# zhaotudou/HeteroFusionRCNN

Measured on AMD Instinct MI355X. Metric: KITTI frames/sec RPN train step, higher is better.
Workload: dtype f32; 1 GPU; RPN train step, hf/configs/rpn_multiclass.config: PointCNN 5 xconv (K=8; 16384/4096/1024/256/64 points; C 256..1024, X-transformation, global branch) + 6 xdconv layers + fc 256/256, 3 classes, seg head, projection of the points into the image + gather of the image feature map (B,360,1200,32) + path drop 0.9/0.9 + 'concat' fusion, bin-based box head (fc 512/512, 3x76 outputs), targets + focal/softm; frames_per_gpu=8, global_batch=8, parallelism=dp1, hip_graph=True, optimizer=hf, x_branch_on_side_stream=True, scaling=strong, library_gemm_selection=library default heuristic, gradient_exchange=none (1 rank), geometry_prefetch_depth=2, geometry_prefetch_group=12

## Files before the change

heterofusionrcnn_amd/csrc/xconv.hip:

```cpp
#include "hf_common.h"

#include <initializer_list>

namespace hf {

template <int M>
__device__ __forceinline__ void store_m(float *base, size_t elem, const float (&v)[M])
{
    float *p = base + elem;
    if constexpr (M == 4 || M == 8) {
        if ((reinterpret_cast<uintptr_t>(base) & 15) == 0) {
#pragma unroll
            for (int q = 0; q < M / 4; ++q) reinterpret_cast<float4 *>(p)[q] = make_float4(v[4 * q], v[4 * q + 1], v[4 * q + 2], v[4 * q + 3]);
            return;
        }
    } else if constexpr (M == 2) {
        if ((reinterpret_cast<uintptr_t>(base) & 7) == 0) { *reinterpret_cast<float2 *>(p) = make_float2(v[0], v[1]); return; }
    }
#pragma unroll
    for (int m = 0; m < M; ++m) p[m] = v[m];
}
template <int M>
__device__ __forceinline__ void load_m(const float *base, size_t elem, float (&v)[M])
{
    const float *p = base + elem;
    if constexpr (M == 4 || M == 8) {
        if ((reinterpret_cast<uintptr_t>(base) & 15) == 0) {
#pragma unroll
            for (int q = 0; q < M / 4; ++q) {
                const float4 t = reinterpret_cast<const float4 *>(p)[q];
                v[4 * q] = t.x; v[4 * q + 1] = t.y; v[4 * q + 2] = t.z; v[4 * q + 3] = t.w;
            }
            return;
        }
    } else if constexpr (M == 2) {
        if ((reinterpret_cast<uintptr_t>(base) & 7) == 0) { const float2 t = *reinterpret_cast<const float2 *>(p); v[0] = t.x; v[1] = t.y; return; }
    }
#pragma unroll
    for (int m = 0; m < M; ++m) v[m] = p[m];
}


constexpr int kXcThreads = 256;

template <int K, bool TRANSPOSED>
__global__ __launch_bounds__(kXcThreads) void xconv_apply_kernel(long long rows, int c, const float *__restrict__ x,
                                                                const float *__restrict__ f, float *__restrict__ out)
{
    const int lane = threadIdx.x & 63;
    const long long wave = __builtin_amdgcn_readfirstlane(static_cast<int>(threadIdx.x >> 6)) +
                           static_cast<long long>(blockIdx.x) * (kXcThreads / 64);
    const long long nwaves = static_cast<long long>(gridDim.x) * (kXcThreads / 64);
    for (long long r = wave; r < rows; r += nwaves) {
        const float *xr = x + r * (K * K);
        float coef[K][K];
#pragma unroll
        for (int i = 0; i < K; ++i)
#pragma unroll
            for (int j = 0; j < K; ++j) coef[i][j] = TRANSPOSED ? xr[j * K + i] : xr[i * K + j];
        const float *fr = f + r * K * c;
        float *orow = out + r * K * c;
        for (int ch = lane; ch < c; ch += 64) {
            float v[K];
#pragma unroll
            for (int j = 0; j < K; ++j) v[j] = fr[static_cast<size_t>(j) * c + ch];
#pragma unroll
            for (int i = 0; i < K; ++i) {
                float acc = coef[i][0] * v[0];
#pragma unroll
                for (int j = 1; j < K; ++j) acc = acc + coef[i][j] * v[j];
                orow[static_cast<size_t>(i) * c + ch] = acc;
            }
        }
    }
}

template <int K>
__global__ __launch_bounds__(kXcThreads) void xconv_dx_kernel(long long rows, int c, const float *__restrict__ grad_out,
                                                             const float *__restrict__ f, float *__restrict__ grad_x)
{
    extern __shared__ float lds[];
    constexpr int KK = K * K, STRIDE = KK + 1;
    const int lane = threadIdx.x & 63, w = threadIdx.x >> 6;
    float *mine = lds + static_cast<size_t>(w) * 64 * STRIDE;
    const long long wave = w + static_cast<long long>(blockIdx.x) * (kXcThreads / 64);
    const long long nwaves = static_cast<long long>(gridDim.x) * (kXcThreads / 64);
    for (long long r = wave; r < rows; r += nwaves) {
        const float *gr = grad_out + r * K * c;
        const float *fr = f + r * K * c;
        float acc[K][K];
#pragma unroll
        for (int i = 0; i < K; ++i)
#pragma unroll
            for (int j = 0; j < K; ++j) acc[i][j] = 0.f;
        for (int ch = lane; ch < c; ch += 64) {
            float g[K], v[K];
#pragma unroll
            for (int j = 0; j < K; ++j) { g[j] = gr[static_cast<size_t>(j) * c + ch]; v[j] = fr[static_cast<size_t>(j) * c + ch]; }
#pragma unroll
            for (int i = 0; i < K; ++i)
#pragma unroll
                for (int j = 0; j < K; ++j) acc[i][j] = acc[i][j] + g[i] * v[j];
        }
#pragma unroll
        for (int i = 0; i < K; ++i)
#pragma unroll
            for (int j = 0; j < K; ++j) mine[lane * STRIDE + i * K + j] = acc[i][j];
        __builtin_amdgcn_fence(__ATOMIC_SEQ_CST, "wavefront");
        __builtin_amdgcn_wave_barrier();
        for (int p = lane; p < KK; p += 64) {
            float s = 0.f;
            for (int l = 0; l < 64; ++l) s = s + mine[l * STRIDE + p];
            grad_x[r * KK + p] = s;
        }
        __builtin_amdgcn_fence(__ATOMIC_SEQ_CST, "wavefront");
        __builtin_amdgcn_wave_barrier();
    }
}

template <int K, int M>
__global__ __launch_bounds__(kXcThreads) void depthwise_fwd_kernel(long long rows, int c, const float *__restrict__ x,
                                                                  const float *__restrict__ wgt, float *__restrict__ y)
{
    const long long total = rows * c;
    for (long long g = static_cast<long long>(blockIdx.x) * kXcThreads + threadIdx.x; g < total;
         g += static_cast<long long>(gridDim.x) * kXcThreads) {
        const long long r = g / c;
        const int ch = static_cast<int>(g - r * c);
        float acc[M];
#pragma unroll
        for (int m = 0; m < M; ++m) acc[m] = 0.f;
#pragma unroll
        for (int w = 0; w < K; ++w) {
            const float xv = x[(r * K + w) * c + ch];
#pragma unroll
            for (int m = 0; m < M; ++m) acc[m] = acc[m] + xv * wgt[(static_cast<size_t>(w) * c + ch) * M + m];
        }
        store_m<M>(y, static_cast<size_t>(g) * M, acc);
    }
}

template <int K, int M>
__global__ __launch_bounds__(kXcThreads) void depthwise_dx_kernel(long long rows, int c, const float *__restrict__ grad_y,
                                                                 const float *__restrict__ wgt, float *__restrict__ grad_x)
{
    const long long total = rows * c;
    for (long long g = static_cast<long long>(blockIdx.x) * kXcThreads + threadIdx.x; g < total;
         g += static_cast<long long>(gridDim.x) * kXcThreads) {
        const long long r = g / c;
        const int ch = static_cast<int>(g - r * c);
        float gy[M];
        load_m<M>(grad_y, static_cast<size_t>(g) * M, gy);
#pragma unroll
        for (int w = 0; w < K; ++w) {
            float acc = 0.f;
#pragma unroll
            for (int m = 0; m < M; ++m) acc = acc + gy[m] * wgt[(static_cast<size_t>(w) * c + ch) * M + m];
            grad_x[(r * K + w) * c + ch] = acc;
        }
    }
}

template <int K, int M, bool DX>
__global__ __launch_bounds__(kXcThreads) void depthwise_narrow_kernel(long long rows, int c, const float *__restrict__ in,
                                                                     const float *__restrict__ wgt, float *__restrict__ out)
{
    const long long tid = static_cast<long long>(blockIdx.x) * kXcThreads + threadIdx.x;
    const long long nthreads = static_cast<long long>(gridDim.x) * kXcThreads;
    const int ch = static_cast<int>(tid % c);
    float wr[K][M];
#pragma unroll
    for (int w = 0; w < K; ++w)
#pragma unroll
        for (int m = 0; m < M; ++m) wr[w][m] = wgt[(static_cast<size_t>(w) * c + ch) * M + m];
    for (long long r = tid / c; r < rows; r += nthreads / c) {
        if (!DX) {
            float acc[M];
#pragma unroll
            for (int m = 0; m < M; ++m) acc[m] = 0.f;
#pragma unroll
            for (int w = 0; w < K; ++w) {
                const float xv = in[(r * K + w) * c + ch];
#pragma unroll
                for (int m = 0; m < M; ++m) acc[m] = acc[m] + xv * wr[w][m];
            }
            store_m<M>(out, static_cast<size_t>(r * c + ch) * M, acc);
        } else {
            float gy[M];
            load_m<M>(in, static_cast<size_t>(r * c + ch) * M, gy);
#pragma unroll
            for (int w = 0; w < K; ++w) {
                float acc = 0.f;
#pragma unroll
                for (int m = 0; m < M; ++m) acc = acc + gy[m] * wr[w][m];
                out[(r * K + w) * c + ch] = acc;
            }
        }
    }
}

static int narrow_grid(long long rows, int c)
{
    int a = c, b = kXcThreads;
    while (b) { const int tmp = a % b; a = b; b = tmp; }
    const int unit = c / a;
    long long g = (rows * c + kXcThreads - 1) / kXcThreads;
    const long long cap = static_cast<long long>(kNumCU) * 8;
    if (g > cap) g = cap;
    g = (g + unit - 1) / unit * unit;
    return static_cast<int>(g);
}
constexpr int kNarrowMaxC = 64;

template <int K, int M>
__global__ __launch_bounds__(kXcThreads) void depthwise_dw_kernel(long long rows, int c, int rows_per_chunk,
                                                                 const float *__restrict__ x, const float *__restrict__ grad_y,
                                                                 float *__restrict__ grad_w, float *__restrict__ partial)
{
    extern __shared__ float red[];
    const int cw = c < kXcThreads ? c : kXcThreads, nrs = kXcThreads / cw;
    const int t = static_cast<int>(threadIdx.x);
    const int cl = t % cw, ch = blockIdx.x * cw + cl, rs = t / cw;
    const bool live = ch < c && rs < nrs;
    if (nrs > 1) {
        for (int i = t; i < K * M * cw; i += kXcThreads) red[i] = 0.f;
        __syncthreads();
    }
    const long long r0 = static_cast<long long>(blockIdx.y) * rows_per_chunk + rs;
    const long long r1 = static_cast<long long>(blockIdx.y + 1) * rows_per_chunk < rows ? static_cast<long long>(blockIdx.y + 1) * rows_per_chunk : rows;
    float acc[K][M];
#pragma unroll
    for (int w = 0; w < K; ++w)
#pragma unroll
        for (int m = 0; m < M; ++m) acc[w][m] = 0.f;
    if (live) {
        for (long long r = r0; r < r1; r += nrs) {
            float gy[M];
            load_m<M>(grad_y, static_cast<size_t>(r * c + ch) * M, gy);
#pragma unroll
            for (int w = 0; w < K; ++w) {
                const float xv = x[(r * K + w) * c + ch];
#pragma unroll
                for (int m = 0; m < M; ++m) acc[w][m] = acc[w][m] + xv * gy[m];
            }
        }
    }
    float *mine = partial ? partial + static_cast<size_t>(blockIdx.y) * K * c * M : nullptr;
    if (nrs == 1) {
        if (live) {
#pragma unroll
            for (int w = 0; w < K; ++w)
#pragma unroll
                for (int m = 0; m < M; ++m) {
                    const size_t e = (static_cast<size_t>(w) * c + ch) * M + m;
                    if (mine) mine[e] = acc[w][m];
                    else atomicAdd(&grad_w[e], acc[w][m]);
                }
        }
        return;
    }
    const bool shuffle = (cw & (cw - 1)) == 0 && cw <= 32;
    if (shuffle) {
        const int lane = t & 63, wave = t >> 6;
        __syncthreads();
#pragma unroll
        for (int w = 0; w < K; ++w)
#pragma unroll
            for (int m = 0; m < M; ++m) {
                float v = live ? acc[w][m] : 0.f;
                for (int off = cw; off < 64; off <<= 1) v += __shfl_xor(v, off);
                if (lane < cw) red[(wave * K * M + w * M + m) * cw + lane] = v;
            }
        __syncthreads();
        for (int i = t; i < K * M * cw; i += kXcThreads) {
            float v = red[i];
#pragma unroll
            for (int wv = 1; wv < kXcThreads / 64; ++wv) v += red[wv * K * M * cw + i];
            const int wm = i / cw, c2 = blockIdx.x * cw + i % cw;
            if (c2 < c) {
                const size_t e = (static_cast<size_t>(wm / M) * c + c2) * M + wm % M;
                if (mine) mine[e] = v;
                else atomicAdd(&grad_w[e], v);
            }
        }
        return;
    }
    if (live) {
#pragma unroll
        for (int w = 0; w < K; ++w)
#pragma unroll
            for (int m = 0; m < M; ++m) atomicAdd(&red[(w * M + m) * cw + cl], acc[w][m]);
    }
    __syncthreads();
    for (int i = t; i < K * M * cw; i += kXcThreads) {
        const int wm = i / cw, c2 = blockIdx.x * cw + i % cw;
        if (c2 < c) {
            const size_t e = (static_cast<size_t>(wm / M) * c + c2) * M + wm % M;
            if (mine) mine[e] = red[i];
            else atomicAdd(&grad_w[e], red[i]);
        }
    }
}

typedef float f2 __attribute__((ext_vector_type(2)));

struct XcPair {
    const float *base;
    unsigned hi;
    bool gathered, live, hi_live;
};

__device__ __forceinline__ XcPair xc_pair(int ch, int c, int c0, const float *f, const float *fts, bool gather)
{
    XcPair s;
    s.live = ch < c;
    s.hi_live = ch + 1 < c;
    const int cc = s.live ? ch : (c - 1) & ~1;
    s.hi = s.hi_live ? 1u : 0u;
    s.gathered = gather && cc >= c0;
    s.base = s.gathered ? fts + (cc - c0) : f + cc;
    return s;
}

template <bool V2>
__device__ __forceinline__ f2 ld_pair(const float *p, unsigned hi)
{
    if constexpr (V2) return *reinterpret_cast<const f2 *>(p);
    else return f2{p[0], p[hi]};
}

template <int M, bool V2>
__device__ __forceinline__ void st_pair_m(float *p, bool hi_live, const f2 (&v)[M])
{
    if constexpr (V2) {
#pragma unroll
        for (int q = 0; q < M; ++q) {
            const int e0 = 2 * q, e1 = 2 * q + 1;
            reinterpret_cast<f2 *>(p)[q] = f2{e0 < M ? v[e0].x : v[e0 - M].y, e1 < M ? v[e1].x : v[e1 - M].y};
        }
    } else {
#pragma unroll
        for (int m = 0; m < M; ++m) p[m] = v[m].x;
        if (hi_live) {
#pragma unroll
            for (int m = 0; m < M; ++m) p[M + m] = v[m].y;
        }
    }
}

constexpr int kXcRows = 2;

struct XcCloud {
    long long next;
    unsigned tbase;
};

__device__ __forceinline__ unsigned xc_tbase(XcCloud &cl, long long r, int rows_per_cloud, int n_src)
{
    while (r >= cl.next) { cl.next += rows_per_cloud; cl.tbase += static_cast<unsigned>(n_src); }
    return cl.tbase;
}

__device__ __forceinline__ XcCloud xc_cloud(long long r, int rows_per_cloud, int n_src)
{
    const long long b = r / rows_per_cloud;
    return XcCloud{(b + 1) * rows_per_cloud, static_cast<unsigned>(b * n_src)};
}

template <int K, bool GATHER, bool V2>
__device__ __forceinline__ void xc_gather_row(const XcPair &s, long long r, unsigned tbase, const int *__restrict__ idx,
                                              unsigned lstride, unsigned c1, f2 (&fv)[K])
{
    const unsigned rk = static_cast<unsigned>(r) * K;
#pragma unroll
    for (int j = 0; j < K; ++j) {
        const unsigned lo = (rk + j) * lstride;
        unsigned off = lo;
        if constexpr (GATHER) {
            const unsigned go = (tbase + static_cast<unsigned>(idx[rk + j])) * c1;
            off = s.gathered ? go : lo;
        }
        fv[j] = ld_pair<V2>(s.base + off, s.hi);
    }
}

template <int K>
struct XcXRows {
    static constexpr int KK = K * K, Q = (KK + 63) / 64;
    float v[kXcRows][Q];
    __device__ __forceinline__ void load(const float *__restrict__ x, const long long (&rr)[kXcRows], int lane)
    {
#pragma unroll
        for (int i = 0; i < kXcRows; ++i)
#pragma unroll
            for (int q = 0; q < Q; ++q) {
                const int p = lane + 64 * q;
                v[i][q] = x[rr[i] * KK + (p < KK ? p : KK - 1)];
            }
    }
    __device__ __forceinline__ void stage(float (*xs)[KK], int lane) const
    {
        __builtin_amdgcn_fence(__ATOMIC_SEQ_CST, "wavefront");
        __builtin_amdgcn_wave_barrier();
#pragma unroll
        for (int i = 0; i < kXcRows; ++i)
#pragma unroll
            for (int q = 0; q < Q; ++q)
                if (lane + 64 * q < KK) xs[i][lane + 64 * q] = v[i][q];
        __builtin_amdgcn_fence(__ATOMIC_SEQ_CST, "wavefront");
        __builtin_amdgcn_wave_barrier();
    }
};

template <int K, int M, bool GATHER, bool V2>
__global__ __launch_bounds__(kXcThreads) void xconv_dw_fwd_kernel(long long rows, int c, int c0, int rows_per_block,
                                                                 const float *__restrict__ x, const float *__restrict__ f,
                                                                 const float *__restrict__ fts, const int *__restrict__ idx, int n_src,
                                                                 int rows_per_cloud, const float *__restrict__ wd, float *__restrict__ out)
{
    const int lane = threadIdx.x & 63, wave = __builtin_amdgcn_readfirstlane(static_cast<int>(threadIdx.x >> 6));
    const int ch = blockIdx.y * 128 + 2 * lane;
    const XcPair src = xc_pair(ch, c, c0, f, fts, GATHER);
    const int cw = src.live ? ch : (c - 1) & ~1;
    f2 w[K][M];
#pragma unroll
    for (int k = 0; k < K; ++k)
#pragma unroll
        for (int m = 0; m < M; ++m) w[k][m] = f2{wd[(static_cast<size_t>(k) * c + cw) * M + m], wd[(static_cast<size_t>(k) * c + cw + src.hi) * M + m]};
    const unsigned lstride = GATHER ? c0 : c, c1 = c - c0;
    const long long r0 = static_cast<long long>(blockIdx.x) * rows_per_block;
    const long long r1 = r0 + rows_per_block < rows ? r0 + rows_per_block : rows;
    __shared__ float xs[kXcThreads / 64][kXcRows][K * K];
    XcCloud cl = xc_cloud(r0, rows_per_cloud, n_src);
    for (long long rb = r0 + wave; rb < r1; rb += 4 * kXcRows) {
        f2 fv[kXcRows][K];
        long long rr[kXcRows];
#pragma unroll
        for (int i = 0; i < kXcRows; ++i) rr[i] = rb + 4 * i < r1 ? rb + 4 * i : r1 - 1;
        XcXRows<K> xrow;
        xrow.load(x, rr, lane);
#pragma unroll
        for (int i = 0; i < kXcRows; ++i) {
            const unsigned tb = GATHER ? xc_tbase(cl, rr[i], rows_per_cloud, n_src) : 0u;
            xc_gather_row<K, GATHER, V2>(src, rr[i], tb, idx, lstride, c1, fv[i]);
        }
        xrow.stage(xs[wave], lane);
#pragma unroll
        for (int i = 0; i < kXcRows; ++i) {
            if (rb + 4 * i >= r1) break;
            const float *xr = xs[wave][i];
            f2 o[M];
#pragma unroll
            for (int m = 0; m < M; ++m) o[m] = f2{0.f, 0.f};
#pragma unroll
            for (int k = 0; k < K; ++k) {
                f2 t = xr[k * K] * fv[i][0];
#pragma unroll
                for (int j = 1; j < K; ++j) t = t + xr[k * K + j] * fv[i][j];
#pragma unroll
                for (int m = 0; m < M; ++m) o[m] = o[m] + t * w[k][m];
            }
            if (src.live) st_pair_m<M, V2>(out + static_cast<size_t>(rr[i] * c + ch) * M, src.hi_live, o);
        }
    }
}

struct XcSource {
    const float *base;
    long long stride;
    bool gathered;
};

__device__ __forceinline__ XcSource xc_source(int ch, int c, int c0, const float *f, const float *fts, const int *idx)
{
    XcSource s;
    if (idx == nullptr) { s.base = f + ch; s.stride = c; s.gathered = false; }
    else if (ch - (ch & 63) < c0) { s.base = f + ch; s.stride = c0; s.gathered = false; }
    else { s.base = fts + (ch - c0); s.stride = c - c0; s.gathered = true; }
    return s;
}

template <int K, int M, bool GATHER>
__global__ __launch_bounds__(kXcThreads) void xconv_dw_bwd_fw_kernel(long long rows, int c, int c0, int rows_per_block,
                                                                    const float *__restrict__ x, const float *__restrict__ f,
                                                                    const float *__restrict__ fts, const int *__restrict__ idx, int n_src,
                                                                    int rows_per_cloud, const float *__restrict__ wd,
                                                                    const float *__restrict__ grad_out, float *__restrict__ grad_f,
                                                                    float *__restrict__ grad_gathered, float *__restrict__ grad_wd,
                                                                    float *__restrict__ wd_partial)
{
    const int lane = threadIdx.x & 63, wave = __builtin_amdgcn_readfirstlane(static_cast<int>(threadIdx.x >> 6));
    const int ch = blockIdx.y * 64 + lane;
    const bool live = ch < c;
    const XcSource src = xc_source(live ? ch : blockIdx.y * 64, c, c0, f, fts, GATHER ? idx : nullptr);
    if (GATHER && src.gathered && !grad_wd && !grad_gathered) return;
    float w[K][M], gw[K][M];
#pragma unroll
    for (int k = 0; k < K; ++k)
#pragma unroll
        for (int m = 0; m < M; ++m) { w[k][m] = live ? wd[(static_cast<size_t>(k) * c + ch) * M + m] : 0.f; gw[k][m] = 0.f; }
    const long long r0 = static_cast<long long>(blockIdx.x) * rows_per_block;
    const long long r1 = r0 + rows_per_block < rows ? r0 + rows_per_block : rows;
    for (long long r = r0 + wave; r < r1; r += kXcThreads / 64) {
        const float *xr = x + r * (K * K);
        float fv[K], g[M], gfx[K];
        const long long tbase = (GATHER && src.gathered) ? static_cast<long long>(static_cast<unsigned>(r) / static_cast<unsigned>(rows_per_cloud)) * n_src : 0;
#pragma unroll
        for (int j = 0; j < K; ++j) {
            const long long srow = (GATHER && src.gathered) ? tbase + idx[r * K + j] : r * K + j;
            fv[j] = live ? src.base[srow * src.stride] : 0.f;
        }
        load_m<M>(grad_out, static_cast<size_t>(r * c + (live ? ch : 0)) * M, g);
        if (!live) {
#pragma unroll
            for (int m = 0; m < M; ++m) g[m] = 0.f;
        }
#pragma unroll
        for (int k = 0; k < K; ++k) {
            float a = 0.f;
#pragma unroll
            for (int m = 0; m < M; ++m) a = a + g[m] * w[k][m];
            gfx[k] = a;
            float t = xr[k * K] * fv[0];
#pragma unroll
            for (int j = 1; j < K; ++j) t = t + xr[k * K + j] * fv[j];
#pragma unroll
            for (int m = 0; m < M; ++m) gw[k][m] = gw[k][m] + t * g[m];
        }
        float *gdst = (GATHER && src.gathered) ? (grad_gathered ? grad_gathered + (ch - c0) : nullptr) : (grad_f ? grad_f + ch : nullptr);
        if (live && gdst) {
#pragma unroll
            for (int j = 0; j < K; ++j) {
                float a = xr[j] * gfx[0];
#pragma unroll
                for (int k = 1; k < K; ++k) a = a + xr[k * K + j] * gfx[k];
                gdst[(r * K + j) * src.stride] = a;
            }
        }
    }
    if (grad_wd) {
        __shared__ float red[K * M][64];
        for (int i = threadIdx.x; i < K * M * 64; i += kXcThreads) (&red[0][0])[i] = 0.f;
        __syncthreads();
        if (live) {
#pragma unroll
            for (int k = 0; k < K; ++k)
#pragma unroll
                for (int m = 0; m < M; ++m) atomicAdd(&red[k * M + m][lane], gw[k][m]);
        }
        __syncthreads();
        float *mine = wd_partial ? wd_partial + static_cast<size_t>(blockIdx.x) * K * c * M : nullptr;
        for (int i = threadIdx.x; i < K * M * 64; i += kXcThreads) {
            const int km = i >> 6, c2 = blockIdx.y * 64 + (i & 63);
            if (c2 < c) {
                const size_t e = (static_cast<size_t>(km / M) * c + c2) * M + km % M;
                if (mine) mine[e] = red[km][i & 63];
                else atomicAdd(&grad_wd[e], red[km][i & 63]);
            }
        }
    }
}

template <int K, int M, bool GATHER>
__global__ __launch_bounds__(kXcThreads) void xconv_dw_bwd_x_kernel(long long rows, int c, int c0, const float *__restrict__ f,
                                                                   const float *__restrict__ fts, const int *__restrict__ idx, int n_src,
                                                                   int rows_per_cloud, const float *__restrict__ wd,
                                                                   const float *__restrict__ grad_out, float *__restrict__ grad_x)
{
    extern __shared__ float lds[];
    constexpr int KK = K * K, STRIDE = KK + 1, QUADS = 16;
    const int lane = threadIdx.x & 63, w = threadIdx.x >> 6;
    float *mine = lds + static_cast<size_t>(w) * QUADS * STRIDE;
    const long long wave = w + static_cast<long long>(blockIdx.x) * (kXcThreads / 64);
    const long long nwaves = static_cast<long long>(gridDim.x) * (kXcThreads / 64);
    const int c1 = c - c0;
    for (long long r = wave; r < rows; r += nwaves) {
        float acc[K][K];
#pragma unroll
        for (int i = 0; i < K; ++i)
#pragma unroll
            for (int j = 0; j < K; ++j) acc[i][j] = 0.f;
        long long trow[K];
        if constexpr (GATHER) {
            const long long tbase = static_cast<long long>(static_cast<unsigned>(r) / static_cast<unsigned>(rows_per_cloud)) * n_src;
#pragma unroll
            for (int j = 0; j < K; ++j) trow[j] = tbase + idx[r * K + j];
        }
        for (int ch = lane; ch < c; ch += 64) {
            float fv[K], g[M];
            if constexpr (GATHER) {
                const bool gathered = ch >= c0;
                const float *base = gathered ? fts + (ch - c0) : f + ch;
                const long long stride = gathered ? c1 : c0;
#pragma unroll
                for (int j = 0; j < K; ++j) fv[j] = base[(gathered ? trow[j] : r * K + j) * stride];
            } else {
#pragma unroll
                for (int j = 0; j < K; ++j) fv[j] = f[(r * K + j) * c + ch];
            }
            load_m<M>(grad_out, static_cast<size_t>(r * c + ch) * M, g);
#pragma unroll
            for (int k = 0; k < K; ++k) {
                float a = 0.f;
#pragma unroll
                for (int m = 0; m < M; ++m) a = a + g[m] * wd[(static_cast<size_t>(k) * c + ch) * M + m];
#pragma unroll
                for (int j = 0; j < K; ++j) acc[k][j] = acc[k][j] + a * fv[j];
            }
        }
#pragma unroll
        for (int i = 0; i < K; ++i)
#pragma unroll
            for (int j = 0; j < K; ++j) {
                float v = acc[i][j];
                v = v + __int_as_float(__builtin_amdgcn_mov_dpp(__float_as_int(v), 0xb1, 0xf, 0xf, true));
                v = v + __int_as_float(__builtin_amdgcn_mov_dpp(__float_as_int(v), 0x4e, 0xf, 0xf, true));
                if ((lane & 3) == 0) mine[(lane >> 2) * STRIDE + i * K + j] = v;
            }
        __builtin_amdgcn_fence(__ATOMIC_SEQ_CST, "wavefront");
        __builtin_amdgcn_wave_barrier();
        for (int p = lane; p < KK; p += 64) {
            float s = 0.f;
#pragma unroll
            for (int l = 0; l < QUADS; ++l) s = s + mine[l * STRIDE + p];
            grad_x[r * KK + p] = s;
        }
        __builtin_amdgcn_fence(__ATOMIC_SEQ_CST, "wavefront");
        __builtin_amdgcn_wave_barrier();
    }
}

template <int K, int M>
__global__ __launch_bounds__(kXcThreads) void xconv_dw_bwd_fts_kernel(long long src_rows, int n_src, long long rows_per_cloud,
                                                                     int c, int c0, int rows_per_block,
                                                                     const float *__restrict__ x, const float *__restrict__ wd,
                                                                     const float *__restrict__ grad_out,
                                                                     const int *__restrict__ offsets, const int *__restrict__ entries,
                                                                     float *__restrict__ grad_fts)
{
    const int lane = threadIdx.x & 63, wave = __builtin_amdgcn_readfirstlane(static_cast<int>(threadIdx.x >> 6));
    const int c1 = c - c0, cf = blockIdx.y * 64 + lane, ch = c0 + cf;
    const bool live = cf < c1;
    float w[K][M];
#pragma unroll
    for (int k = 0; k < K; ++k)
#pragma unroll
        for (int m = 0; m < M; ++m) w[k][m] = live ? wd[(static_cast<size_t>(k) * c + ch) * M + m] : 0.f;
    const long long s0 = static_cast<long long>(blockIdx.x) * rows_per_block;
    const long long s1 = s0 + rows_per_block < src_rows ? s0 + rows_per_block : src_rows;
    long long bb = s0 / n_src;
    for (long long s = s0 + wave; s < s1; s += kXcThreads / 64) {
        while (s >= (bb + 1) * n_src) ++bb;
        const int pt = static_cast<int>(s - bb * n_src);
        const int *off = offsets + bb * (n_src + 1);
        const int *ent = entries + bb * rows_per_cloud * K;
        const int lo = off[pt], hi = off[pt + 1];
        float acc = 0.f;
        for (int e = lo; e < hi; e += 4) {
            float a4[4];
#pragma unroll
            for (int u = 0; u < 4; ++u) {
                const bool valid = e + u < hi;
                const int slot = ent[valid ? e + u : lo];
                const long long r = bb * rows_per_cloud + slot / K;
                const int j = slot % K;
                const float *xr = x + r * (K * K);
                float g[M], gfx[K];
                load_m<M>(grad_out, static_cast<size_t>(r * c + (live ? ch : 0)) * M, g);
                if (!live) {
#pragma unroll
                    for (int m = 0; m < M; ++m) g[m] = 0.f;
                }
#pragma unroll
                for (int k = 0; k < K; ++k) {
                    float a = 0.f;
#pragma unroll
                    for (int m = 0; m < M; ++m) a = a + g[m] * w[k][m];
                    gfx[k] = a;
                }
                float a = xr[j] * gfx[0];
#pragma unroll
                for (int k = 1; k < K; ++k) a = a + xr[k * K + j] * gfx[k];
                a4[u] = valid ? a : 0.f;
            }
#pragma unroll
            for (int u = 0; u < 4; ++u) acc += a4[u];
        }
        if (live) grad_fts[s * c1 + cf] = acc;
    }
}

static int grid_for(long long items, int per_block)
{
    const long long blocks = (items + per_block - 1) / per_block;
    return static_cast<int>(blocks < 1 ? 1 : (blocks > 8 * kNumCU ? 8 * kNumCU : blocks));
}

template <int K>
static int launch_apply(long long rows, int c, const float *x, const float *f, float *out, bool transposed, hipStream_t st)
{
    const int grid = grid_for(rows, kXcThreads / 64);
    if (transposed) hipLaunchKernelGGL((xconv_apply_kernel<K, true>), dim3(grid), dim3(kXcThreads), 0, st, rows, c, x, f, out);
    else hipLaunchKernelGGL((xconv_apply_kernel<K, false>), dim3(grid), dim3(kXcThreads), 0, st, rows, c, x, f, out);
    return launch_status();
}

template <int K>
static int launch_dx(long long rows, int c, const float *grad_out, const float *f, float *grad_x, hipStream_t st)
{
    const size_t lds = sizeof(float) * (kXcThreads / 64) * 64 * (K * K + 1);
    const int lrc = ensure_dynamic_lds(reinterpret_cast<const void *>(&xconv_dx_kernel<K>), lds);
    if (lrc != HF_OK) return lrc;
    hipLaunchKernelGGL((xconv_dx_kernel<K>), dim3(grid_for(rows, kXcThreads / 64)), dim3(kXcThreads), lds, st, rows, c, grad_out, f,
                       grad_x);
    return launch_status();
}

}

using namespace hf;

HF_API int hf_xconv_apply(long long rows, int k, int c, const float *x, const float *f, float *out, hf_stream_t stream)
{
    if (rows < 0 || c <= 0 || !x || !f || !out) return HF_EINVAL;
    if (rows == 0) return HF_OK;
    switch (k) {
    case 4: return launch_apply<4>(rows, c, x, f, out, false, as_stream(stream));
    case 8: return launch_apply<8>(rows, c, x, f, out, false, as_stream(stream));
    default: return HF_EINVAL;
    }
}

HF_API int hf_xconv_apply_grad(long long rows, int k, int c, const float *x, const float *f, const float *grad_out,
                               float *grad_x, float *grad_f, hf_stream_t stream)
{
    if (rows < 0 || c <= 0 || !x || !f || !grad_out || (!grad_x && !grad_f)) return HF_EINVAL;
    if (rows == 0) return HF_OK;
    hipStream_t st = as_stream(stream);
    int rc = HF_OK;
#define HF_XC_CASE(KK)                                                                                                 \
    case KK:                                                                                                           \
        if (grad_f) rc = launch_apply<KK>(rows, c, x, grad_out, grad_f, true, st);                                     \
        if (rc == HF_OK && grad_x) rc = launch_dx<KK>(rows, c, grad_out, f, grad_x, st);                               \
        return rc;
    switch (k) {
        HF_XC_CASE(4)
        HF_XC_CASE(8)
    default: return HF_EINVAL;
    }
#undef HF_XC_CASE
}

#define HF_DW_DISPATCH(CALL)                                                                                           \
    if (k == 8 && m == 1) { CALL(8, 1) } else if (k == 8 && m == 2) { CALL(8, 2) } else if (k == 8 && m == 3) { CALL(8, 3) }      \
    else if (k == 8 && m == 4) { CALL(8, 4) } else if (k == 8 && m == 8) { CALL(8, 8) }                                 \
    else if (k == 4 && m == 1) { CALL(4, 1) } else if (k == 4 && m == 4) { CALL(4, 4) }                                 \
    else return HF_EINVAL;

HF_API int hf_depthwise_k(long long rows, int k, int c, int m, const float *x, const float *w, float *y, hf_stream_t stream)
{
    if (rows < 0 || c <= 0 || !x || !w || !y) return HF_EINVAL;
    if (rows == 0) return HF_OK;
    if (c <= kNarrowMaxC && k * m <= 64) {
        const int ng = narrow_grid(rows, c);
#define HF_DW_NFWD(KK, MM) hipLaunchKernelGGL((depthwise_narrow_kernel<KK, MM, false>), dim3(ng), dim3(kXcThreads), 0, as_stream(stream), rows, c, x, w, y);
        HF_DW_DISPATCH(HF_DW_NFWD)
#undef HF_DW_NFWD
        return launch_status();
    }
    const int grid = grid_for(rows * c, kXcThreads);
#define HF_DW_FWD(KK, MM) hipLaunchKernelGGL((depthwise_fwd_kernel<KK, MM>), dim3(grid), dim3(kXcThreads), 0, as_stream(stream), rows, c, x, w, y);
    HF_DW_DISPATCH(HF_DW_FWD)
#undef HF_DW_FWD
    return launch_status();
}

static void dw_chunks(long long rows, int c, int &cblocks, int &rows_per_chunk, unsigned &nchunks)
{
    cblocks = c < kXcThreads ? 1 : div_up(c, kXcThreads);
    long long chunks = (2 * kNumCU + cblocks - 1) / cblocks;
    if (chunks > (rows + 63) / 64) chunks = (rows + 63) / 64;
    if (chunks < 1) chunks = 1;
    if (chunks > rows) chunks = rows;
    if (chunks > 65535) chunks = 65535;
    rows_per_chunk = static_cast<int>((rows + chunks - 1) / chunks);
    nchunks = static_cast<unsigned>((rows + rows_per_chunk - 1) / rows_per_chunk);
}

HF_API size_t hf_depthwise_k_grad_workspace(long long rows, int k, int c, int m)
{
    if (rows <= 0 || k <= 0 || c <= 0 || m <= 0) return 0;
    int cblocks, rpc;
    unsigned nchunks;
    dw_chunks(rows, c, cblocks, rpc, nchunks);
    return sizeof(float) * static_cast<size_t>(nchunks) * k * c * m;
}

static int depthwise_k_grad_impl(long long rows, int k, int c, int m, const float *x, const float *w, const float *grad_y,
                                 float *grad_x, float *grad_w, float *partial, hipStream_t st)
{
    if (grad_w && (!partial || rows == 0)) {
        const int rc = hip_status(hipMemsetAsync(grad_w, 0, sizeof(float) * static_cast<size_t>(k) * c * m, st));
        if (rc != HF_OK) return rc;
    }
    if (rows == 0) return HF_OK;
    if (grad_x && c <= kNarrowMaxC && k * m <= 64) {
        const int ng = narrow_grid(rows, c);
#define HF_DW_NDX(KK, MM) hipLaunchKernelGGL((depthwise_narrow_kernel<KK, MM, true>), dim3(ng), dim3(kXcThreads), 0, st, rows, c, grad_y, w, grad_x);
        HF_DW_DISPATCH(HF_DW_NDX)
#undef HF_DW_NDX
        const int rc = launch_status();
        if (rc != HF_OK) return rc;
    } else if (grad_x) {
        const int grid = grid_for(rows * c, kXcThreads);
#define HF_DW_DX(KK, MM) hipLaunchKernelGGL((depthwise_dx_kernel<KK, MM>), dim3(grid), dim3(kXcThreads), 0, st, rows, c, grad_y, w, grad_x);
        HF_DW_DISPATCH(HF_DW_DX)
#undef HF_DW_DX
        const int rc = launch_status();
        if (rc != HF_OK) return rc;
    }
    if (grad_w) {
        int cblocks, rows_per_chunk;
        unsigned nchunks;
        dw_chunks(rows, c, cblocks, rows_per_chunk, nchunks);
        const size_t lds = c <= kXcThreads / 2 ? sizeof(float) * static_cast<size_t>(k) * m * c * (((c & (c - 1)) == 0 && c <= 32) ? kXcThreads / 64 : 1) : 0;
        if (lds > 48 * 1024) return HF_EINVAL;
        const dim3 grid(cblocks, nchunks);
#define HF_DW_DW(KK, MM) hipLaunchKernelGGL((depthwise_dw_kernel<KK, MM>), grid, dim3(kXcThreads), lds, st, rows, c, rows_per_chunk, x, grad_y, grad_w, partial);
        HF_DW_DISPATCH(HF_DW_DW)
#undef HF_DW_DW
        if (partial) launch_partial_reduce(k * c * m, static_cast<int>(nchunks), partial, grad_w, st);
        return launch_status();
    }
    return HF_OK;
}

HF_API int hf_depthwise_k_grad(long long rows, int k, int c, int m, const float *x, const float *w, const float *grad_y,
                               float *grad_x, float *grad_w, hf_stream_t stream)
{
    if (rows < 0 || c <= 0 || !x || !w || !grad_y || (!grad_x && !grad_w)) return HF_EINVAL;
    return depthwise_k_grad_impl(rows, k, c, m, x, w, grad_y, grad_x, grad_w, nullptr, as_stream(stream));
}

HF_API int hf_depthwise_k_grad_ws(long long rows, int k, int c, int m, const float *x, const float *w, const float *grad_y,
                                  float *grad_x, float *grad_w, void *workspace, size_t workspace_bytes, hf_stream_t stream)
{
    if (rows < 0 || c <= 0 || !x || !w || !grad_y || (!grad_x && !grad_w)) return HF_EINVAL;
    if (grad_w && rows > 0 && (!workspace || workspace_bytes < hf_depthwise_k_grad_workspace(rows, k, c, m))) return HF_EWORKSPACE;
    return depthwise_k_grad_impl(rows, k, c, m, x, w, grad_y, grad_x, grad_w, grad_w ? static_cast<float *>(workspace) : nullptr,
                                 as_stream(stream));
}

#define HF_XDW_DISPATCH(CALL)                                                                                          \
    if (k == 8 && m == 1) { CALL(8, 1) } else if (k == 8 && m == 2) { CALL(8, 2) } else if (k == 8 && m == 3) { CALL(8, 3) }      \
    else if (k == 8 && m == 4) { CALL(8, 4) }                                                                          \
    else if (k == 4 && m == 1) { CALL(4, 1) } else if (k == 4 && m == 4) { CALL(4, 4) }    \
    else if (k == 12 && m == 1) { CALL(12, 1) } else if (k == 12 && m == 2) { CALL(12, 2) }                             \
    else return HF_EINVAL;

static void xdw_grid(long long rows, int c, dim3 &grid, int &rows_per_block, int blocks_per_cu = 8, int chunk = 64)
{
    const int cchunks = div_up(c, chunk);
    long long rchunks = (blocks_per_cu * kNumCU + cchunks - 1) / cchunks;
    if (rchunks > (rows + 3) / 4) rchunks = (rows + 3) / 4;
    if (rchunks < 1) rchunks = 1;
    rows_per_block = static_cast<int>((rows + rchunks - 1) / rchunks);
    grid = dim3(static_cast<unsigned>((rows + rows_per_block - 1) / rows_per_block), cchunks);
}

static bool xdw_offsets_fit(long long rows, int k, int c, long long src_rows)
{
    return rows * k * static_cast<long long>(c) < (1ll << 32) && src_rows * static_cast<long long>(c) < (1ll << 32);
}

static bool xdw_v2(int c, std::initializer_list<const void *> ptrs)
{
    if (c & 1) return false;
    for (const void *p : ptrs)
        if (reinterpret_cast<uintptr_t>(p) & 7) return false;
    return true;
}

static void xdw_pair_grid(long long rows, int c, dim3 &grid, int &rpb, int blocks_per_cu) { xdw_grid(rows, c, grid, rpb, blocks_per_cu, 128); }

static int xdw_forward(long long rows, int k, int c, int c0, int m, const float *x, const float *f, const float *fts, const int *idx,
                       int n_src, int rows_per_cloud, const float *wd, float *out, hipStream_t st)
{
    if (!xdw_offsets_fit(rows, k, c, idx ? static_cast<long long>(rows / rows_per_cloud) * n_src : 0)) return HF_EINVAL;
    dim3 grid;
    int rpb;
    xdw_pair_grid(rows, c, grid, rpb, 8);
    const bool v2 = xdw_v2(c, {f, fts, out});
#define HF_XDW_FWD_V(KK, MM, V)                                                                                        \
    if (idx) hipLaunchKernelGGL((xconv_dw_fwd_kernel<KK, MM, true, V>), grid, dim3(kXcThreads), 0, st, rows, c, c0, rpb, x, f, fts, idx, n_src, rows_per_cloud, wd, out); \
    else hipLaunchKernelGGL((xconv_dw_fwd_kernel<KK, MM, false, V>), grid, dim3(kXcThreads), 0, st, rows, c, c0, rpb, x, f, fts, idx, n_src, rows_per_cloud, wd, out);
#define HF_XDW_FWD(KK, MM) if (v2) { HF_XDW_FWD_V(KK, MM, true) } else { HF_XDW_FWD_V(KK, MM, false) }
    HF_XDW_DISPATCH(HF_XDW_FWD)
#undef HF_XDW_FWD
#undef HF_XDW_FWD_V
    return launch_status();
}

static void xdw_bwd_grid(long long rows, int c, dim3 &grid, int &rpb)
{
    xdw_grid(rows, c, grid, rpb, 4);
    if (rpb < 32 && rows > 32) { rpb = 32; grid.x = static_cast<unsigned>((rows + rpb - 1) / rpb); }
}

static int xdw_backward(long long rows, int k, int c, int c0, int m, const float *x, const float *f, const float *fts, const int *idx,
                        int n_src, int rows_per_cloud, const float *wd, const float *grad_out, float *grad_x, float *grad_f, float *grad_gathered,
                        float *grad_wd, hipStream_t st, float *wd_partial = nullptr)
{
    if (grad_wd && (!wd_partial || rows == 0)) {
        const int rc = hip_status(hipMemsetAsync(grad_wd, 0, sizeof(float) * static_cast<size_t>(k) * c * m, st));
        if (rc != HF_OK) return rc;
    }
    if (rows == 0) return HF_OK;
    if (!grad_wd) wd_partial = nullptr;
    if (grad_f || grad_wd || grad_gathered) {
        dim3 grid;
        int rpb;
        xdw_bwd_grid(rows, c, grid, rpb);
#define HF_XDW_BFW(KK, MM)                                                                                             \
        if (idx) hipLaunchKernelGGL((xconv_dw_bwd_fw_kernel<KK, MM, true>), grid, dim3(kXcThreads), 0, st, rows, c, c0, rpb, x, f, fts, idx, n_src, rows_per_cloud, wd, grad_out, grad_f, grad_gathered, grad_wd, wd_partial); \
        else hipLaunchKernelGGL((xconv_dw_bwd_fw_kernel<KK, MM, false>), grid, dim3(kXcThreads), 0, st, rows, c, c0, rpb, x, f, fts, idx, n_src, rows_per_cloud, wd, grad_out, grad_f, grad_gathered, grad_wd, wd_partial);
        HF_XDW_DISPATCH(HF_XDW_BFW)
#undef HF_XDW_BFW
        if (wd_partial) launch_partial_reduce(k * c * m, static_cast<int>(grid.x), wd_partial, grad_wd, st);
        const int rc = launch_status();
        if (rc != HF_OK) return rc;
    }
    if (grad_x) {
        const size_t lds = sizeof(float) * (kXcThreads / 64) * 16 * (static_cast<size_t>(k) * k + 1);
#define HF_XDW_BX(KK, MM)                                                                                              \
        if (idx) hipLaunchKernelGGL((xconv_dw_bwd_x_kernel<KK, MM, true>), dim3(grid_for(rows, kXcThreads / 64)), dim3(kXcThreads), lds, st, rows, c, c0, f, fts, idx, n_src, rows_per_cloud, wd, grad_out, grad_x); \
        else hipLaunchKernelGGL((xconv_dw_bwd_x_kernel<KK, MM, false>), dim3(grid_for(rows, kXcThreads / 64)), dim3(kXcThreads), lds, st, rows, c, c0, f, fts, idx, n_src, rows_per_cloud, wd, grad_out, grad_x);
        HF_XDW_DISPATCH(HF_XDW_BX)
#undef HF_XDW_BX
        return launch_status();
    }
    return HF_OK;
}

HF_API int hf_xconv_depthwise(long long rows, int k, int c, int m, const float *x, const float *f, const float *wd, float *out,
                              hf_stream_t stream)
{
    if (rows < 0 || c <= 0 || !x || !f || !wd || !out) return HF_EINVAL;
    if (rows == 0) return HF_OK;
    return xdw_forward(rows, k, c, c, m, x, f, nullptr, nullptr, 0, 1, wd, out, as_stream(stream));
}

HF_API int hf_xconv_depthwise_grad(long long rows, int k, int c, int m, const float *x, const float *f, const float *wd,
                                   const float *grad_out, float *grad_x, float *grad_f, float *grad_wd, hf_stream_t stream)
{
    if (rows < 0 || c <= 0 || !x || !f || !wd || !grad_out || (!grad_x && !grad_f && !grad_wd)) return HF_EINVAL;
    return xdw_backward(rows, k, c, c, m, x, f, nullptr, nullptr, 0, 1, wd, grad_out, grad_x, grad_f, nullptr, grad_wd, as_stream(stream));
}

HF_API int hf_xconv_depthwise_gather(int b, int n_src, int rows_per_cloud, int k, int c0, int c1, int m, const float *x,
                                     const float *f_delta, const float *fts, const int *idx, const float *wd, float *out,
                                     hf_stream_t stream)
{
    if (b < 0 || n_src <= 0 || rows_per_cloud < 0 || c0 <= 0 || c0 % 64 != 0 || c1 <= 0) return HF_EINVAL;
    const long long rows = static_cast<long long>(b) * rows_per_cloud;
    if (rows == 0) return HF_OK;
    if (rows > 0x7fffffffll || !x || !f_delta || !fts || !idx || !wd || !out) return HF_EINVAL;
    return xdw_forward(rows, k, c0 + c1, c0, m, x, f_delta, fts, idx, n_src, rows_per_cloud, wd, out, as_stream(stream));
}

static size_t xdw_gathered_bytes(int b, int rows_per_cloud, int k, int c1)
{
    return (sizeof(float) * static_cast<size_t>(b) * rows_per_cloud * k * c1 + 255) & ~static_cast<size_t>(255);
}

HF_API size_t hf_xconv_depthwise_gather_grad_workspace(int b, int rows_per_cloud, int k, int c0, int c1, int m)
{
    if (b <= 0 || rows_per_cloud <= 0 || k <= 0 || c0 <= 0 || c1 <= 0 || m <= 0) return 0;
    dim3 grid;
    int rpb;
    xdw_bwd_grid(static_cast<long long>(b) * rows_per_cloud, c0 + c1, grid, rpb);
    return xdw_gathered_bytes(b, rows_per_cloud, k, c1) + sizeof(float) * static_cast<size_t>(grid.x) * k * (c0 + c1) * m;
}

HF_API int hf_xconv_depthwise_gather_grad(int b, int n_src, int rows_per_cloud, int k, int c0, int c1, int m, const float *x,
                                          const float *f_delta, const float *fts, const int *idx, const float *wd,
                                          const float *grad_out, const int *offsets, const int *entries, float *grad_x,
                                          float *grad_f_delta, float *grad_fts, float *grad_wd, void *workspace,
                                          size_t workspace_bytes, hf_stream_t stream)
{
    if (b < 0 || n_src <= 0 || rows_per_cloud < 0 || c0 <= 0 || c0 % 64 != 0 || c1 <= 0 || !x || !f_delta || !fts || !idx || !wd ||
        !grad_out || static_cast<long long>(b) * rows_per_cloud > 0x7fffffffll ||
        (!grad_x && !grad_f_delta && !grad_fts && !grad_wd))
        return HF_EINVAL;
    if (grad_fts && (!offsets || !entries)) return HF_EINVAL;
    if (workspace && workspace_bytes < hf_xconv_depthwise_gather_grad_workspace(b, rows_per_cloud, k, c0, c1, m)) return HF_EWORKSPACE;
    hipStream_t st = as_stream(stream);
    const long long rows = static_cast<long long>(b) * rows_per_cloud;
    const int c = c0 + c1;
    float *gathered = (grad_fts && workspace) ? static_cast<float *>(workspace) : nullptr;
    float *wd_partial = workspace ? reinterpret_cast<float *>(static_cast<unsigned char *>(workspace) + xdw_gathered_bytes(b, rows_per_cloud, k, c1)) : nullptr;
    if (grad_x || grad_f_delta || grad_wd || gathered) {
        const int rc = xdw_backward(rows, k, c, c0, m, x, f_delta, fts, idx, n_src, rows_per_cloud, wd, grad_out, grad_x, grad_f_delta, gathered,
                                    grad_wd, st, wd_partial);
        if (rc != HF_OK) return rc;
    }
    if (grad_fts) {
        const long long src_rows = static_cast<long long>(b) * n_src;
        if (src_rows == 0) return HF_OK;
        if (rows == 0) return hip_status(hipMemsetAsync(grad_fts, 0, sizeof(float) * static_cast<size_t>(src_rows) * c1, st));
        if (gathered) return hf_group_point_grad_gather(b, n_src, c1, rows_per_cloud, k, c1, 0, gathered, offsets, entries, grad_fts, stream);
        dim3 grid;
        int rpb;
        xdw_grid(src_rows, c1, grid, rpb);
#define HF_XDW_FTS(KK, MM) hipLaunchKernelGGL((xconv_dw_bwd_fts_kernel<KK, MM>), grid, dim3(kXcThreads), 0, st, src_rows, n_src, static_cast<long long>(rows_per_cloud), c, c0, rpb, x, wd, grad_out, offsets, entries, grad_fts);
        HF_XDW_DISPATCH(HF_XDW_FTS)
#undef HF_XDW_FTS
        return launch_status();
    }
    return HF_OK;
}
```

Measured before the change: 303.9 frames/s.

## Restructure depthwise X-conv fts gradient kernel and route by size heuristic

Rewrites the direct grad_fts kernel so each wave handles two source rows and four entries at a time. Each lane now covers two or four channels with packed float2 math and vectorized grad_out loads. X-transform rows are staged cooperatively through shared memory, and slot indices for the next step are prefetched. A heuristic chooses between this direct path and the staged gather-then-reduce path based on fanout and staged-buffer size, which can skip the large intermediate write. The cost is higher register pressure, a new grid shape assumption in xdw_grid, and possible divergence when entry counts differ between rows.

```diff
diff --git a/heterofusionrcnn_amd/csrc/xconv.hip b/heterofusionrcnn_amd/csrc/xconv.hip
--- a/heterofusionrcnn_amd/csrc/xconv.hip
+++ b/heterofusionrcnn_amd/csrc/xconv.hip
@@ -630,63 +630,175 @@
     }
 }
 
-template <int K, int M>
+constexpr int kFtsRows = 2, kFtsEntries = 4;
+typedef float f4 __attribute__((ext_vector_type(4)));
+
+constexpr int xc_fts_pairs(int m) { return m == 1 ? 2 : 1; }
+
+template <int K, int M, bool VEC>
 __global__ __launch_bounds__(kXcThreads) void xconv_dw_bwd_fts_kernel(long long src_rows, int n_src, long long rows_per_cloud,
                                                                      int c, int c0, int rows_per_block,
                                                                      const float *__restrict__ x, const float *__restrict__ wd,
-                                                                     const float *__restrict__ grad_out,
+                                                                     const float *grad_out,
                                                                      const int *__restrict__ offsets, const int *__restrict__ entries,
-                                                                     float *__restrict__ grad_fts)
-{
+                                                                     float *grad_fts)
+{
+    constexpr int NP = xc_fts_pairs(M), CPL = 2 * NP, T = kFtsRows, E = kFtsEntries, NF = CPL * M, CHUNK = NF % 4 == 0 ? 4 : 2;
+    constexpr int KP = K <= 4 ? 4 : (K <= 8 ? 8 : 16), QPL = 64 / KP, NR = (T * E + QPL - 1) / QPL;
     const int lane = threadIdx.x & 63, wave = __builtin_amdgcn_readfirstlane(static_cast<int>(threadIdx.x >> 6));
-    const int c1 = c - c0, cf = blockIdx.y * 64 + lane, ch = c0 + cf;
-    const bool live = cf < c1;
-    float w[K][M];
+    const int lq = lane / KP, lk = lane % KP < K ? lane % KP : K - 1;
+    const int c1 = c - c0, col0 = blockIdx.y * (64 * CPL), cf0 = col0 + lane * CPL;
+    unsigned cc[CPL];
+    bool live[CPL];
+#pragma unroll
+    for (int i = 0; i < CPL; ++i) {
+        live[i] = cf0 + i < c1;
+        cc[i] = static_cast<unsigned>(c0 + (live[i] ? cf0 + i : (VEC ? col0 + i : c1 - 1)));
+    }
+    f2 w[K][NP][M];
 #pragma unroll
     for (int k = 0; k < K; ++k)
 #pragma unroll
-        for (int m = 0; m < M; ++m) w[k][m] = live ? wd[(static_cast<size_t>(k) * c + ch) * M + m] : 0.f;
+        for (int p = 0; p < NP; ++p)
+#pragma unroll
+            for (int m = 0; m < M; ++m)
+                w[k][p][m] = f2{wd[(static_cast<size_t>(k) * c + cc[2 * p]) * M + m], wd[(static_cast<size_t>(k) * c + cc[2 * p + 1]) * M + m]};
+    __shared__ __attribute__((aligned(16))) float xs[kXcThreads / 64][T * E][KP];
     const long long s0 = static_cast<long long>(blockIdx.x) * rows_per_block;
     const long long s1 = s0 + rows_per_block < src_rows ? s0 + rows_per_block : src_rows;
     long long bb = s0 / n_src;
-    for (long long s = s0 + wave; s < s1; s += kXcThreads / 64) {
-        while (s >= (bb + 1) * n_src) ++bb;
-        const int pt = static_cast<int>(s - bb * n_src);
-        const int *off = offsets + bb * (n_src + 1);
-        const int *ent = entries + bb * rows_per_cloud * K;
-        const int lo = off[pt], hi = off[pt + 1];
-        float acc = 0.f;
-        for (int e = lo; e < hi; e += 4) {
-            float a4[4];
-#pragma unroll
-            for (int u = 0; u < 4; ++u) {
-                const bool valid = e + u < hi;
-                const int slot = ent[valid ? e + u : lo];
-                const long long r = bb * rows_per_cloud + slot / K;
-                const int j = slot % K;
-                const float *xr = x + r * (K * K);
-                float g[M], gfx[K];
-                load_m<M>(grad_out, static_cast<size_t>(r * c + (live ? ch : 0)) * M, g);
-                if (!live) {
-#pragma unroll
-                    for (int m = 0; m < M; ++m) g[m] = 0.f;
+    for (long long sb = s0 + wave * T; sb < s1; sb += (kXcThreads / 64) * T) {
+        int pos[T], hi[T];
+        long long ebase[T];
+        unsigned rbase[T];
+        f2 acc[T][NP];
+        bool more = false;
+#pragma unroll
+        for (int t = 0; t < T; ++t) {
+            const long long s = sb + t < s1 ? sb + t : s1 - 1;
+            while (s >= (bb + 1) * n_src) ++bb;
+            const int pt = static_cast<int>(s - bb * n_src);
+            const int *off = offsets + bb * (n_src + 1);
+            ebase[t] = bb * rows_per_cloud * K;
+            rbase[t] = static_cast<unsigned>(bb * rows_per_cloud);
+            pos[t] = off[pt];
+            hi[t] = sb + t < s1 ? off[pt + 1] : pos[t];
+            more = more || pos[t] < hi[t];
+#pragma unroll
+            for (int p = 0; p < NP; ++p) acc[t][p] = f2{0.f, 0.f};
+        }
+        auto load_slots = [&](int ahead, unsigned (&slot)[NR]) {
+#pragma unroll
+            for (int i = 0; i < NR; ++i) {
+                const int q = i * QPL + lq < T * E ? i * QPL + lq : T * E - 1, u = q % E + ahead;
+                int e = 0;
+                long long eb = 0;
+#pragma unroll
+                for (int t = 0; t < T; ++t)
+                    if (q / E == t) { e = pos[t] + u < hi[t] ? pos[t] + u : 0; eb = ebase[t]; }
+                slot[i] = static_cast<unsigned>(entries[eb + e]);
+            }
+        };
+        unsigned slot[NR], slot_next[NR];
+        if (more) load_slots(0, slot);
+        while (more) {
+            unsigned rr[T * E];
+            float xv[NR];
+#pragma unroll
+            for (int i = 0; i < NR; ++i) {
+                const int q = i * QPL + lq < T * E ? i * QPL + lq : T * E - 1;
+                unsigned rb = 0;
+#pragma unroll
+                for (int t = 0; t < T; ++t)
+                    if (q / E == t) rb = rbase[t];
+                xv[i] = x[static_cast<size_t>(rb + slot[i] / K) * (K * K) + lk * K + slot[i] % K];
+#pragma unroll
+                for (int j = 0; j < QPL; ++j) {
+                    const int qj = i * QPL + j;
+                    if (qj < T * E) rr[qj] = rbase[qj / E] + static_cast<unsigned>(__builtin_amdgcn_readlane(static_cast<int>(slot[i]), j * KP)) / K;
                 }
-#pragma unroll
-                for (int k = 0; k < K; ++k) {
-                    float a = 0.f;
-#pragma unroll
-                    for (int m = 0; m < M; ++m) a = a + g[m] * w[k][m];
-                    gfx[k] = a;
+            }
+            f2 g[T * E][NP][M];
+#pragma unroll
+            for (int q = 0; q < T * E; ++q) {
+                const float *gp = grad_out + static_cast<size_t>(rr[q]) * c * M;
+                if constexpr (VEC) {
+                    float flat[NF];
+#pragma unroll
+                    for (int i = 0; i < NF / CHUNK; ++i) {
+                        if constexpr (CHUNK == 4) {
+                            const f4 v = *reinterpret_cast<const f4 *>(gp + cc[0] * M + 4 * i);
+                            flat[4 * i] = v.x; flat[4 * i + 1] = v.y; flat[4 * i + 2] = v.z; flat[4 * i + 3] = v.w;
+                        } else {
+                            const f2 v = *reinterpret_cast<const f2 *>(gp + cc[0] * M + 2 * i);
+                            flat[2 * i] = v.x; flat[2 * i + 1] = v.y;
+                        }
+                    }
+#pragma unroll
+                    for (int p = 0; p < NP; ++p)
+#pragma unroll
+                        for (int m = 0; m < M; ++m) g[q][p][m] = f2{flat[2 * p * M + m], flat[(2 * p + 1) * M + m]};
+                } else {
+#pragma unroll
+                    for (int p = 0; p < NP; ++p)
+#pragma unroll
+                        for (int m = 0; m < M; ++m) g[q][p][m] = f2{gp[cc[2 * p] * M + m], gp[cc[2 * p + 1] * M + m]};
                 }
-                float a = xr[j] * gfx[0];
-#pragma unroll
-                for (int k = 1; k < K; ++k) a = a + xr[k * K + j] * gfx[k];
-                a4[u] = valid ? a : 0.f;
-            }
-#pragma unroll
-            for (int u = 0; u < 4; ++u) acc += a4[u];
-        }
-        if (live) grad_fts[s * c1 + cf] = acc;
+            }
+            load_slots(E, slot_next);
+            __builtin_amdgcn_fence(__ATOMIC_SEQ_CST, "wavefront");
+            __builtin_amdgcn_wave_barrier();
+#pragma unroll
+            for (int i = 0; i < NR; ++i) xs[wave][i * QPL + lq < T * E ? i * QPL + lq : T * E - 1][lane % KP] = xv[i];
+            __builtin_amdgcn_fence(__ATOMIC_SEQ_CST, "wavefront");
+            __builtin_amdgcn_wave_barrier();
+            more = false;
+#pragma unroll
+            for (int t = 0; t < T; ++t) {
+#pragma unroll
+                for (int u = 0; u < E; ++u) {
+                    const int q = t * E + u;
+                    if (pos[t] + u >= hi[t]) continue;
+                    const float *xr = xs[wave][q];
+#pragma unroll
+                    for (int p = 0; p < NP; ++p) {
+                        f2 gfx[K];
+#pragma unroll
+                        for (int k = 0; k < K; ++k) {
+                            f2 a = f2{0.f, 0.f};
+#pragma unroll
+                            for (int m = 0; m < M; ++m) a = a + g[q][p][m] * w[k][p][m];
+                            gfx[k] = a;
+                        }
+                        f2 a = xr[0] * gfx[0];
+#pragma unroll
+                        for (int k = 1; k < K; ++k) a = a + xr[k] * gfx[k];
+                        acc[t][p] = acc[t][p] + a;
+                    }
+                }
+                pos[t] += E;
+                more = more || pos[t] < hi[t];
+            }
+#pragma unroll
+            for (int i = 0; i < NR; ++i) slot[i] = slot_next[i];
+        }
+#pragma unroll
+        for (int t = 0; t < T; ++t) {
+            if (sb + t >= s1) break;
+            float *dst = grad_fts + static_cast<size_t>(sb + t) * c1 + cf0;
+            if constexpr (VEC) {
+                if (live[0]) {
+                    if constexpr (NP == 2) *reinterpret_cast<f4 *>(dst) = f4{acc[t][0].x, acc[t][0].y, acc[t][1].x, acc[t][1].y};
+                    else *reinterpret_cast<f2 *>(dst) = acc[t][0];
+                }
+            } else {
+#pragma unroll
+                for (int p = 0; p < NP; ++p) {
+                    if (live[2 * p]) dst[2 * p] = acc[t][p].x;
+                    if (live[2 * p + 1]) dst[2 * p + 1] = acc[t][p].y;
+                }
+            }
+        }
     }
 }
 
@@ -968,6 +1080,29 @@
     return xdw_forward(rows, k, c0 + c1, c0, m, x, f_delta, fts, idx, n_src, rows_per_cloud, wd, out, as_stream(stream));
 }
 
+static bool xdw_fts_direct(long long rows, int n_src, int rows_per_cloud, int k, int c1, int m)
+{
+    if (static_cast<long long>(rows_per_cloud) * k >= 8ll * n_src) return true;
+    const long long staged = rows * k * c1 * static_cast<long long>(sizeof(float));
+    return staged <= (8ll << 20) || (m <= 2 && staged >= (80ll << 20));
+}
+
+static int xdw_table_grad(long long src_rows, int n_src, int rows_per_cloud, int k, int c, int c0, int m, const float *x, const float *wd,
+                          const float *grad_out, const int *offsets, const int *entries, float *grad_fts, hipStream_t st)
+{
+    const int c1 = c - c0, cpl = 2 * xc_fts_pairs(m);
+    dim3 grid;
+    int rpb;
+    xdw_grid(src_rows, c1, grid, rpb, 8, 64 * cpl);
+    const bool vec = c1 % cpl == 0 && ((reinterpret_cast<uintptr_t>(grad_out) | reinterpret_cast<uintptr_t>(grad_fts)) & 15) == 0;
+#define HF_XDW_FTS_V(KK, MM, V) hipLaunchKernelGGL((xconv_dw_bwd_fts_kernel<KK, MM, V>), grid, dim3(kXcThreads), 0, st, src_rows, n_src, static_cast<long long>(rows_per_cloud), c, c0, rpb, x, wd, grad_out, offsets, entries, grad_fts);
+#define HF_XDW_FTS(KK, MM) if (vec) { HF_XDW_FTS_V(KK, MM, true) } else { HF_XDW_FTS_V(KK, MM, false) }
+    HF_XDW_DISPATCH(HF_XDW_FTS)
+#undef HF_XDW_FTS
+#undef HF_XDW_FTS_V
+    return launch_status();
+}
+
 static size_t xdw_gathered_bytes(int b, int rows_per_cloud, int k, int c1)
 {
     return (sizeof(float) * static_cast<size_t>(b) * rows_per_cloud * k * c1 + 255) & ~static_cast<size_t>(255);
@@ -995,27 +1130,23 @@
     if (grad_fts && (!offsets || !entries)) return HF_EINVAL;
     if (workspace && workspace_bytes < hf_xconv_depthwise_gather_grad_workspace(b, rows_per_cloud, k, c0, c1, m)) return HF_EWORKSPACE;
     hipStream_t st = as_stream(stream);
-    const long long rows = static_cast<long long>(b) * rows_per_cloud;
+    const long long rows = static_cast<long long>(b) * rows_per_cloud, src_rows = static_cast<long long>(b) * n_src;
     const int c = c0 + c1;
-    float *gathered = (grad_fts && workspace) ? static_cast<float *>(workspace) : nullptr;
+    const bool want_fts = grad_fts && src_rows > 0 && rows > 0;
+    bool direct = want_fts && (!workspace || xdw_fts_direct(rows, n_src, rows_per_cloud, k, c1, m));
+    if (want_fts && workspace && HF_DIAG_INT("HF_XDW_FTS_ROUTE", 0) != 0) direct = HF_DIAG_INT("HF_XDW_FTS_ROUTE", 0) == 2;
+    float *gathered = (want_fts && !direct) ? static_cast<float *>(workspace) : nullptr;
     float *wd_partial = workspace ? reinterpret_cast<float *>(static_cast<unsigned char *>(workspace) + xdw_gathered_bytes(b, rows_per_cloud, k, c1)) : nullptr;
+    if (grad_fts && src_rows > 0 && rows == 0) {
+        const int rc = hip_status(hipMemsetAsync(grad_fts, 0, sizeof(float) * static_cast<size_t>(src_rows) * c1, st));
+        if (rc != HF_OK) return rc;
+    }
     if (grad_x || grad_f_delta || grad_wd || gathered) {
         const int rc = xdw_backward(rows, k, c, c0, m, x, f_delta, fts, idx, n_src, rows_per_cloud, wd, grad_out, grad_x, grad_f_delta, gathered,
                                     grad_wd, st, wd_partial);
         if (rc != HF_OK) return rc;
     }
-    if (grad_fts) {
-        const long long src_rows = static_cast<long long>(b) * n_src;
-        if (src_rows == 0) return HF_OK;
-        if (rows == 0) return hip_status(hipMemsetAsync(grad_fts, 0, sizeof(float) * static_cast<size_t>(src_rows) * c1, st));
-        if (gathered) return hf_group_point_grad_gather(b, n_src, c1, rows_per_cloud, k, c1, 0, gathered, offsets, entries, grad_fts, stream);
-        dim3 grid;
-        int rpb;
-        xdw_grid(src_rows, c1, grid, rpb);
-#define HF_XDW_FTS(KK, MM) hipLaunchKernelGGL((xconv_dw_bwd_fts_kernel<KK, MM>), grid, dim3(kXcThreads), 0, st, src_rows, n_src, static_cast<long long>(rows_per_cloud), c, c0, rpb, x, wd, grad_out, offsets, entries, grad_fts);
-        HF_XDW_DISPATCH(HF_XDW_FTS)
-#undef HF_XDW_FTS
-        return launch_status();
-    }
+    if (gathered) return hf_group_point_grad_gather(b, n_src, c1, rows_per_cloud, k, c1, 0, gathered, offsets, entries, grad_fts, stream);
+    if (direct) return xdw_table_grad(src_rows, n_src, rows_per_cloud, k, c, c0, m, x, wd, grad_out, offsets, entries, grad_fts, st);
     return HF_OK;
 }
```

Measured after the change: 312.5 frames/s, median of 6. 2.8% higher.
